# hitfeelee/rtm3d

Measured on AMD Instinct MI355X. Metric: images_per_sec, higher is better.
Workload: dtype fp16

## Files before the change

rtm3d_amd/csrc/common.h:

```cpp
#pragma once
#include <hip/hip_runtime.h>
#include <stdint.h>
#include <stddef.h>

typedef _Float16 f16;
typedef _Float16 f16x8 __attribute__((ext_vector_type(8)));
typedef _Float16 f16x4 __attribute__((ext_vector_type(4)));
typedef _Float16 f16x2 __attribute__((ext_vector_type(2)));
typedef float f32x4 __attribute__((ext_vector_type(4)));
typedef uint32_t u32x4 __attribute__((ext_vector_type(4)));

__device__ __forceinline__ int div_small_q(int m, int d, float rcp_d) {
    const int q = (int)((float)m * rcp_d);
    const int r = m - q * d;
    return q + (r >= d ? 1 : 0) - (r < 0 ? 1 : 0);
}


#define RT_DMA16(gptr, lds_byte_addr) \
    asm volatile("s_mov_b32 m0, %1\n\ts_nop 0\n\tglobal_load_lds_dwordx4 %0, off" : : "v"(gptr), "s"(lds_byte_addr) : "memory", "m0")
#define RT_DMA16_NT(gptr, lds_byte_addr) \
    asm volatile("s_mov_b32 m0, %1\n\ts_nop 0\n\tglobal_load_lds_dwordx4 %0, off nt" : : "v"(gptr), "s"(lds_byte_addr) : "memory", "m0")
static __device__ __forceinline__ const void* rt_uniform_ptr(const void* p) {
    const unsigned long long v = (unsigned long long)p;
// ... 151 lines not shown
    int in_coff[RT_MAX_GROUPS], out_coff[RT_MAX_GROUPS];
    int tap_pix[RT_MAX_TAPS];
};
struct QuantMx8Args {
    const f16* in;
    uint8_t* out;
    uint8_t* out_s;
    int B, H, W;
    int in_Hp, in_Wp, in_C, in_P, in_coff;
    int out_Hp, out_Wp, out_C, out_P, out_coff;
    int nblk;
};

struct PersistentGrid { int grid, single; };
inline PersistentGrid persistent_grid(int total, int cu_count) { return {cu_count < total ? cu_count : total, total <= cu_count ? 1 : 0}; }

hipError_t launch_patch_mask(const PatchMaskArgs& a, hipStream_t s);
hipError_t launch_conv32s2_fused(const Conv32S2Args& a, int cu_count, unsigned int* ticket_ctr, hipStream_t s);
hipError_t launch_stem_fused(const StemFusedArgs& a, hipStream_t s);
hipError_t launch_conv_headout(const HeadOutArgs& a, hipStream_t s);
hipError_t launch_conv_mfma(const ConvKArgs& a, int bn_tile, int groups, int epi_nchw, hipStream_t s);
hipError_t launch_conv_mfma_deep(const ConvKArgs& a, int bn_tile, int groups, unsigned int* tile_ctr, hipStream_t s);
hipError_t launch_conv_mfma256(const ConvKArgs& a, int groups, unsigned int* tile_ctr, float* stat_out, hipStream_t s);
enum Conv256Route { C256_ONE_TILE, C256_PERSISTENT, C256_HALO, C256_LATTICE };
Conv256Route conv_mfma256_route(const ConvKArgs& a, int groups, HaloTaps* ht);
void conv_mfma256_permute_weights(const f16* src, f16* dst, size_t n_ktiles);
bool conv64_halo_supported(const ConvKArgs& a, int groups);
hipError_t launch_conv64_halo(const ConvKArgs& a, int cu_count, unsigned int* ticket_ctr, hipStream_t s);
hipError_t launch_conv64_root(const ConvKArgs& a, const RootKArgs& r, int cu_count, unsigned int* ticket_ctr, hipStream_t s);
bool conv64s2_halo_supported(const ConvKArgs& a, int groups);
hipError_t launch_conv64s2_halo(const ConvKArgs& a, int cu_count, unsigned int* ticket_ctr, hipStream_t s);
bool conv128_halo_supported(const ConvKArgs& a, int groups);
hipError_t launch_conv128_halo(const ConvKArgs& a, int cu_count, unsigned int* ticket_ctr, hipStream_t s);
hipError_t launch_conv_smallc(const ConvKArgs& a, hipStream_t s);
bool conv_smallc_supported(int cin, int cout, int ntaps);
hipError_t launch_nchw_to_nhwc4(const float* in, f16* out, int B, int H, int W, int Hp, int Wp, int P, hipStream_t s);
hipError_t launch_maxpool(const PoolKArgs& a, hipStream_t s);
hipError_t launch_softmax_fuse(const SoftmaxKArgs& a, hipStream_t s);
hipError_t launch_quant_mx8(const QuantMx8Args& a, hipStream_t s);
hipError_t launch_conv_mx8(const ConvMx8Args& a, int groups, hipStream_t s);
```

rtm3d_amd/csrc/conv128_halo.hip:

```cpp
#include "common.h"

#define LDS_AS __attribute__((address_space(3)))
#define C128_NSW 3
#define C128_DMA16 RT_DMA16
#define C128_LDS_F16X8(byte_addr) (*(const LDS_AS f16x8*)(uintptr_t)(byte_addr))

template <int RES>
__global__ __launch_bounds__(512) void conv128_halo_kernel(const ConvKArgs a, unsigned int* ticket_ctr, const int single) {
    constexpr int TW = 32, CT = 128;
    constexpr int HW = TW + 2;
    constexpr int HALO_PIECES = 10 * HW * 8;
    constexpr int XI = (HALO_PIECES + 511) / 512;
    constexpr int XBUF_PIECES = XI * 512;
    constexpr int WSLOT_PIECES = CT * 8;
    constexpr int WI = WSLOT_PIECES / 512;
    constexpr int WCN = CT / 64;
    constexpr int WPN = 8 / WCN;
    constexpr int ROWS = 8 / WPN;
    __shared__ __attribute__((aligned(128))) f16 lds[(2 * XBUF_PIECES + C128_NSW * WSLOT_PIECES) * 8];
    __shared__ int tk[3];
    const int tid = threadIdx.x;
    const int lane = tid & 63;
    const int wave = __builtin_amdgcn_readfirstlane(tid >> 6);
    const int wc = wave % WCN, wp = wave / WCN;
    const int frow = lane & 15, fk = lane >> 4;
    const ConvGroupArgs& g = a.g[0];

    const int Hm = a.HmWm / a.Wm;
    const int tiles_x = a.Wm / TW, tpi = tiles_x * (Hm >> 3);
    const int NT = a.cout / CT, cpt = a.cpt;
    const int total = (a.M / a.HmWm) * tpi * NT;

    uint32_t poff[XI];
#pragma unroll
    for (int i = 0; i < XI; ++i) {
        int p = i * 512 + tid;
        p = p < HALO_PIECES ? p : HALO_PIECES - 1;
        const int hq = p >> 3, hcs = p & 7;
// ... 9 lines not shown
        cur = blockIdx.x; nxt = nn = total;
    } else {
        if (tid == 0) tk[0] = (int)atomicAdd(ticket_ctr, 3u);
        __syncthreads();
        const int tk0 = __builtin_amdgcn_readfirstlane(tk[0]);
        cur = tk0; nxt = tk0 + 1; nn = tk0 + 2;
    }
    if (cur >= total) return;
    __syncthreads();

    auto halo_origin = [&](int v) -> const f16* {
        const int pt = v / NT;
        const int n = pt / tpi, r = pt - n * tpi;
        const int ty = r / tiles_x, tx = r - ty * tiles_x;
        return a.in + ((size_t)(n * a.in_Hp + ty * 8 - 1 + a.in_P) * a.in_Wp + tx * TW - 1 + a.in_P) * a.in_C + g.in_coff;
    };
    auto issue_x = [&](const f16* src, int xb, int i, uint32_t off) {
        C128_DMA16(src + off, __builtin_amdgcn_readfirstlane(lds_x + (uint32_t)((xb * XBUF_PIECES + i * 512 + wave * 64) * 16)));
    };
    auto issue_w = [&](int nt, int tap, int chunk, int slot) {
        const f16* src = wsrc + (size_t)((nt * 9 + tap) * cpt + chunk) * (CT * 64);
#pragma unroll
        for (int i = 0; i < WI; ++i)
            C128_DMA16(src + i * 512 * 8, __builtin_amdgcn_readfirstlane(lds_w + (uint32_t)((slot * WSLOT_PIECES + i * 512 + wave * 64) * 16)));
    };

    const uint32_t lane_px = (uint32_t)(((ROWS * wp + 1) * HW + frow + 1) * 128);
    const uint32_t ck_m = (uint32_t)((((frow + 0) ^ fk) & 7) << 4), ck_0 = (uint32_t)((((frow + 1) ^ fk) & 7) << 4),
                   ck_p = (uint32_t)((((frow + 2) ^ fk) & 7) << 4);
    const uint32_t lane_w = (uint32_t)((wc * 64 + frow) * 128);
    const uint32_t wk0 = (uint32_t)(((fk ^ (frow & 7)) & 7) << 4), wk1 = (uint32_t)((((4 + fk) ^ (frow & 7)) & 7) << 4);
    const f16 lo = a.relu ? (f16)0.f : (f16)(-__builtin_inff());
    const f16x4 lo4 = {lo, lo, lo, lo};
    const int so = (fk & 1) * 16 + (fk >> 1) * 8;

    {
        const f16* src = halo_origin(cur);
#pragma unroll
        for (int i = 0; i < XI; ++i) issue_x(src, 0, i, poff[i]);
        issue_w(cur % NT, 0, 0, 0);
        issue_w(cur % NT, 1, 0, 1);
    }
    asm volatile("s_waitcnt vmcnt(0)" ::: "memory");

    int it = 0;
    f32x4 acc[4][4];
    for (;;) {
#pragma unroll
        for (int c = 0; c < 4; ++c)
#pragma unroll
            for (int p = 0; p < 4; ++p) acc[c][p] = (f32x4){0.f, 0.f, 0.f, 0.f};
        const bool more = nxt < total;
        const int nt_cur = cur % NT, nt_nxt = more ? nxt % NT : nt_cur;
        const f16* const src_cur = halo_origin(cur);
        const f16* const src_nxt = more ? halo_origin(nxt) : src_cur;
#pragma unroll 1
        for (int chunk = 0; chunk < cpt; ++chunk) {
            const bool last = chunk + 1 == cpt;
            const f16* const src_next = last ? src_nxt : src_cur + 64 * (chunk + 1);
            const int nt_next = last ? nt_nxt : nt_cur, chunk_next = last ? 0 : chunk + 1;
            const int xb = chunk & 1;
            uint32_t hb = lds_x + (uint32_t)(xb * XBUF_PIECES * 16);
            asm volatile("" : "+v"(hb));
#pragma unroll
            for (int t = 0; t < 9; ++t) {
                asm volatile("s_waitcnt vmcnt(%0)" : : "n"(WI + 1) : "memory");
                __builtin_amdgcn_sched_barrier(0);
                __builtin_amdgcn_s_barrier();
                __builtin_amdgcn_sched_barrier(0);
                if (chunk == 0 && t == 0 && it > 0) nn = __builtin_amdgcn_readfirstlane(tk[(it - 1) & 1]);
                {
                    if (t + 2 < 9) issue_w(nt_cur, t + 2, chunk, (t + 2) % C128_NSW);
                    else issue_w(nt_next, t + 2 - 9, chunk_next, (t + 2) % C128_NSW);
                    const int i = t < XI ? t : XI - 1;
                    issue_x(src_next, xb ^ 1, i, poff[i]);
                }
                const int dy = t / 3 - 1, dx = t % 3 - 1;
                const uint32_t ck = dx < 0 ? ck_m : (dx > 0 ? ck_p : ck_0);
                const uint32_t xt0 = hb + lane_px + (uint32_t)((dy * HW + dx) * 128) + ck;
                const uint32_t xu = xt0 ^ (uint32_t)(((1 + dy) & 1) << 6), xw = xu ^ 64u;
                const uint32_t wb = lds_w + (uint32_t)((t % C128_NSW) * WSLOT_PIECES * 16) + lane_w;
                f16x8 xf[2][4], wf[2][4];
#pragma unroll
                for (int kk = 0; kk < 2; ++kk) {
#pragma unroll
                    for (int p = 0; p < 4; ++p) {
                        const int prow = p >> 1, pcol = (p & 1) * 16;
                        const uint32_t ad = (((prow & 1) ^ kk) ? xw : xu) + (uint32_t)((prow * HW + pcol) * 128);
                        xf[kk][p] = C128_LDS_F16X8(ad);
                    }
#pragma unroll
                    for (int c = 0; c < 4; ++c) wf[kk][c] = C128_LDS_F16X8(wb + (uint32_t)(c * 16 * 128) + (kk ? wk1 : wk0));
                }
#pragma unroll
                for (int kk = 0; kk < 2; ++kk)
#pragma unroll
                    for (int c = 0; c < 4; ++c)
#pragma unroll
                        for (int p = 0; p < 4; ++p)
                            acc[c][p] = __builtin_amdgcn_mfma_f32_16x16x32_f16(wf[kk][c], xf[kk][p], acc[c][p], 0, 0, 0);
            }
        }
        if (!single && tid == 0) tk[it & 1] = (int)atomicAdd(ticket_ctr, 1u);

        {
            const int pt = cur / NT;
            const int n = pt / tpi, r = pt - n * tpi;
            const int ty = r / tiles_x, tx = r - ty * tiles_x;
            const int cbase = nt_cur * CT + wc * 64;
            f32x4 bv[4];
#pragma unroll
            for (int c = 0; c < 4; ++c) bv[c] = *(const f32x4*)(a.bias + g.bias_off + cbase + c * 16 + fk * 4);
            size_t opix[4];
            f16x4 rv[4][4];
#pragma unroll
            for (int p = 0; p < 4; ++p) {
                const int prow = p >> 1, pcol = (p & 1) * 16;
                const int oy = ty * 8 + ROWS * wp + prow, ox = tx * TW + pcol + frow;
                opix[p] = ((size_t)(n * a.out_Hp + oy + a.out_P) * a.out_Wp + ox + a.out_P) * a.out_C + g.out_coff + cbase;
                if (RES) {
                    const f16* rp = a.res + ((size_t)(n * a.res_Hp + oy + a.res_P) * a.res_Wp + ox + a.res_P) * a.res_C + g.res_coff + cbase + fk * 4;
#pragma unroll
                    for (int c = 0; c < 4; ++c) rv[p][c] = *(const f16x4*)(rp + c * 16);
                }
            }
#pragma unroll
            for (int p = 0; p < 4; ++p) {
                uint32_t u[4][2];
#pragma unroll
                for (int c = 0; c < 4; ++c) {
                    f32x4 v = acc[c][p] + bv[c];
                    if (RES) {
                        const f16x4 rr = rv[p][c];
                        v[0] += (float)rr[0]; v[1] += (float)rr[1]; v[2] += (float)rr[2]; v[3] += (float)rr[3];
                    }
                    f16x4 h = {(f16)v[0], (f16)v[1], (f16)v[2], (f16)v[3]};
                    h = __builtin_elementwise_max(h, lo4);
                    __builtin_memcpy(u[c], &h, 8);
                }
#pragma unroll
                for (int c = 0; c < 4; c += 2) {
                    const auto s0 = __builtin_amdgcn_permlane16_swap(u[c][0], u[c + 1][0], false, false);
                    const auto s1 = __builtin_amdgcn_permlane16_swap(u[c][1], u[c + 1][1], false, false);
                    const u32x4 o = {s0[0], s1[0], s0[1], s1[1]};
                    *(u32x4*)((f16*)a.out + opix[p] + c * 16 + so) = o;
                }
            }
        }
        if (!more) break;
        cur = nxt; nxt = nn;
        ++it;
    }
}

bool conv128_halo_supported(const ConvKArgs& a, int groups) {
    if (groups != 1 || a.cin % 128 || a.cout % 128 || a.ntaps != 9 || a.in_stride != 1 || a.out_scale != 1 || a.in_P < 1) return false;
    if (a.Wm % 32 || (a.HmWm / a.Wm) % 8 || a.M % a.HmWm) return false;
    const int pitch = a.in_Wp * a.in_C;
    for (int t = 0; t < 9; ++t)
        if (a.g[0].tap_off[t] != (t / 3 - 1) * pitch + (t % 3 - 1) * a.in_C) return false;
    return true;
}

hipError_t launch_conv128_halo(const ConvKArgs& a, int cu_count, unsigned int* ticket_ctr, hipStream_t s) {
    const int total = (a.M / a.HmWm) * (a.Wm >> 5) * ((a.HmWm / a.Wm) >> 3) * (a.cout / 128);
    const auto [grid, single] = persistent_grid(total, cu_count);
    if (a.res) hipLaunchKernelGGL(conv128_halo_kernel<1>, dim3(grid), dim3(512), 0, s, a, ticket_ctr, single);
    else hipLaunchKernelGGL(conv128_halo_kernel<0>, dim3(grid), dim3(512), 0, s, a, ticket_ctr, single);
    return hipGetLastError();
}
```

rtm3d_amd/csrc/conv_mfma256.hip:

```cpp
#include <string.h>
#include "common.h"

#define LDS_AS __attribute__((address_space(3)))
#define GLB_AS __attribute__((address_space(1)))

void conv_mfma256_permute_weights(const f16* src, f16* dst, size_t n_ktiles) {
    for (size_t k = 0; k < n_ktiles; ++k)
        for (int rd = 0; rd < 256; ++rd) {
            const int j = rd >> 7, wc = (rd >> 5) & 3, c = (rd >> 4) & 1, frow = rd & 15;
            const int rs = wc * 64 + frow * 4 + j * 2 + c;
            for (int pos = 0; pos < 8; ++pos) {
                const int chunk = pos ^ (rd & 7);
                memcpy(dst + (k * 256 + rd) * 64 + pos * 8, src + (k * 256 + rs) * 64 + (chunk ^ (rs & 7)) * 8, 16);
            }
        }
}

#define HALF_ELEMS (128 * 64)
#define BUF_ELEMS (4 * HALF_ELEMS)
#define SLOT_XA 0
#define SLOT_XB 1
#define SLOT_WA 2
#define SLOT_WB 3

__device__ __forceinline__ void c256_next_pixel(int& n, int& y, int& x, bool live, int Wm, int Hm) {
    const bool wx = x + 1 == Wm, wy = wx && y + 1 == Hm;
    const int x1 = wx ? 0 : x + 1, y1 = wy ? 0 : (wx ? y + 1 : y), n1 = wy ? n + 1 : n;
    x = live ? x1 : x; y = live ? y1 : y; n = live ? n1 : n;
}

template <int RES>
__global__ __launch_bounds__(512) void conv_mfma256_kernel(const ConvKArgs a) {
    __shared__ __attribute__((aligned(16))) f16 lds[2 * BUF_ELEMS + HALF_ELEMS];
    const int tid = threadIdx.x;
    const int lane = tid & 63;
    const int wave = __builtin_amdgcn_readfirstlane(tid >> 6);
    const int wp = wave & 1, wc = wave >> 1;

    const int bid = blockIdx.x;
    const int xcd = bid & 7, jb = bid >> 3;
    const int chunk = (a.MT + 7) >> 3;
    const int ntile = jb % a.NT;
    const int mtile = xcd * chunk + jb / a.NT;
    if (mtile >= a.MT) return;
    const ConvGroupArgs& g = a.g[blockIdx.y];
    const int T = a.ksteps;

    uint32_t xoff[2][2];
    {
        const int rr = tid >> 3, cs = tid & 7;
#pragma unroll
        for (int h = 0; h < 2; ++h)
#pragma unroll
            for (int i = 0; i < 2; ++i) {
                int m = mtile * 256 + h * 128 + i * 64 + rr;
                m = m < a.M ? m : a.M - 1;
                const int n = m / a.HmWm, rem = m - n * a.HmWm;
                const int y = rem / a.Wm, x = rem - y * a.Wm;
                const uint32_t pix = (uint32_t)((n * a.in_Hp + y * a.in_stride + a.in_P) * a.in_Wp + x * a.in_stride + a.in_P);
                xoff[h][i] = pix * (uint32_t)a.in_C + (uint32_t)g.in_coff + (uint32_t)((cs ^ (rr & 7)) * 8);
            }
    }
    const f16* wbase = a.wgt + g.w_off + (size_t)ntile * T * (256 * 64);
    f16* const dummy = lds + 2 * BUF_ELEMS;
// ... 74 lines not shown
        LOAD_W(wa, buf + SLOT_WA * HALF_ELEMS)
        stage(SLOT_WB, t + 1);
        SEG_SYNC()
        MMA(0, 0, wa)
        LOAD_W(wb, buf + SLOT_WB * HALF_ELEMS)
        stage(SLOT_XB, t + 1);
        SEG_SYNC()
        MMA(0, 1, wb)
        LOAD_X(buf + SLOT_XB * HALF_ELEMS)
        stage(SLOT_XA, t + 2);
        SEG_SYNC()
        MMA(1, 1, wb)
        stage(SLOT_WA, t + 2);
        SEG_SYNC()
        MMA(1, 0, wa)
    }
    if (wave < 4) __builtin_amdgcn_s_barrier();

    const f32x4 bv = *(const f32x4*)(a.bias + g.bias_off + ntile * 256 + wc * 64 + frow * 4);
    const float lo = a.relu ? 0.f : -__builtin_inff();
    const int cbase = ntile * 256 + wc * 64 + frow * 4;
    const int Hm = a.HmWm / a.Wm;
#pragma unroll
    for (int i = 0; i < 2; ++i) {
        size_t opix[4][4];
        f16x4 rv[4][4];
#pragma unroll
        for (int p = 0; p < 4; ++p) {
            const int m0 = mtile * 256 + i * 128 + wp * 64 + p * 16 + fk * 4;
            const int m = m0 < a.M ? m0 : a.M - 1;
            int n = m / a.HmWm;
            const int rem = m - n * a.HmWm;
            int y = rem / a.Wm, x = rem - y * a.Wm;
#pragma unroll
            for (int e = 0; e < 4; ++e) {
                if (e) c256_next_pixel(n, y, x, m0 + e < a.M, a.Wm, Hm);
                const int oy = y * a.out_scale + g.out_oy, ox = x * a.out_scale + g.out_ox;
                opix[p][e] = ((size_t)(n * a.out_Hp + oy + a.out_P) * a.out_Wp + ox + a.out_P) * a.out_C + g.out_coff + cbase;
                if (RES) rv[p][e] = *(const f16x4*)(a.res + ((size_t)(n * a.res_Hp + oy + a.res_P) * a.res_Wp + ox + a.res_P) * a.res_C + g.res_coff + cbase);
            }
        }
#pragma unroll
        for (int p = 0; p < 4; ++p)
#pragma unroll
            for (int e = 0; e < 4; ++e) {
                f32x4 v = {acc[i][0][0][p][e], acc[i][0][1][p][e], acc[i][1][0][p][e], acc[i][1][1][p][e]};
                v += bv;
                if (RES) {
                    const f16x4 r = rv[p][e];
                    v[0] += (float)r[0]; v[1] += (float)r[1]; v[2] += (float)r[2]; v[3] += (float)r[3];
                }
                const f16x4 h = {(f16)fmaxf(v[0], lo), (f16)fmaxf(v[1], lo), (f16)fmaxf(v[2], lo), (f16)fmaxf(v[3], lo)};
                *(f16x4*)((f16*)a.out + opix[p][e]) = h;
            }
    }
}

#define CONV256_MAX_BIAS 2048
#define DMA16 RT_DMA16
#define DMA16_NT RT_DMA16_NT
#define DMA16_SBASE RT_DMA16_SBASE
#define DMA16_SBASE_NT RT_DMA16_SBASE_NT
#define LDS_F16X8(byte_addr) (*(const LDS_AS f16x8*)(uintptr_t)(byte_addr))
#define LOAD_X_N(SLOT)                                                                      \
    _Pragma("unroll") for (int p = 0; p < 4; ++p) {                                         \
        xf[p][0] = LDS_F16X8(xaddr0 + (SLOT) * HALF_ELEMS * 2 + p * 2048);                  \
        xf[p][1] = LDS_F16X8(xaddr1 + (SLOT) * HALF_ELEMS * 2 + p * 2048);                  \
    }
#define LOAD_W_N(dstf, SLOT)                                                                \
    _Pragma("unroll") for (int c = 0; c < 2; ++c) {                                         \
        dstf[c][0] = LDS_F16X8(waddr0 + (SLOT) * HALF_ELEMS * 2 + c * 2048);                \
        dstf[c][1] = LDS_F16X8(waddr1 + (SLOT) * HALF_ELEMS * 2 + c * 2048);                \
// ... 79 lines not shown
    {                                                                                       \
         \
        const uint32_t xaddr0 = opa[0], xaddr1 = opa[1], waddr0 = opa[2], waddr1 = opa[3];  \
        LOAD_X_N(SLOT_XA)                                                                   \
        LOAD_W_N(wa, SLOT_WA)                                                               \
        STAGE_WB_P1                                                                         \
        SEG_SYNC_S(VM1, 0)                                                                  \
        MMA_S(0, 0, wa, FIRST, 1, 0)                                                        \
        LOAD_W_N(wb, SLOT_WB)                                                               \
        stage(SLOT_XB, t + 1, sp ^ 1, koff1);                                               \
        STAGE_WB_P2                                                                         \
        SEG_SYNC_S(VM, 5)                                                                   \
        MMA_S(0, 1, wb, FIRST, 1, 5)                                                        \
        LOAD_X_N(SLOT_XB)                                                                   \
        stage(SLOT_XA, t + 2, sp, koff2);                                                   \
        SEG_SYNC_S(VM, 10)                                                                  \
        MMA_S(1, 1, wb, FIRST, 1, 10)                                                       \
         \
              \
        int kchan3;                                                                         \
        int kraw3 = koff_parts(t + 3, kchan3);                                              \
        stage(SLOT_WA, t + 2, sp, 0);                                                       \
        OPA_SET(sp ^ 1)                                                                     \
        asm volatile("" : "+v"(opa[0]), "+v"(opa[1]), "+v"(opa[2]), "+v"(opa[3]));          \
        STAGE_WB_P4                                                                         \
        SEG_SYNC_S(VM, 15)                                                                  \
        asm volatile("" : "+s"(kraw3));            \
        const int koff3 = kraw3 + kchan3;                                                   \
        MMA_S(1, 0, wa, FIRST, !(LAST), 15)                                                 \
        koff1 = koff2; koff2 = koff3;                                                       \
        sp ^= 1;                                                                            \
    }

template <int RES, int XNT>
__global__ __launch_bounds__(512) void conv_mfma256_persistent_kernel(const ConvKArgs a, const int groups, const int nbias, unsigned int* tile_ctr, const int one_list) {
    __shared__ __attribute__((aligned(16))) f16 lds[2 * BUF_ELEMS + HALF_ELEMS];
    __shared__ __attribute__((aligned(16))) float lds_bias[CONV256_MAX_BIAS + 4];
#ifdef C256_STAMPS
    __shared__ unsigned long long lds_stamp[2][C256_STAMP_KT][C256_STAMP_N];
    __shared__ unsigned long long lds_tstamp[2][4][4];
    int stamp_tile = 0;
#endif
    const int tid = threadIdx.x;
    const int lane = tid & 63;
    const int wave = __builtin_amdgcn_readfirstlane(tid >> 6);
    const int wp = wave & 1, wc = wave >> 1;
    const int T = a.ksteps;
    for (int i = tid; i < nbias; i += 512) lds_bias[i] = a.bias[i];
    __syncthreads();

    const int xcd = one_list ? 0 : blockIdx.x & 7, per_xcd = one_list ? gridDim.x : gridDim.x >> 3;
    const int chunk = one_list ? a.MT : (a.MT + 7) >> 3;
    int mt_here = a.MT - xcd * chunk;
    mt_here = mt_here < 0 ? 0 : (mt_here > chunk ? chunk : mt_here);
    const int jbs = mt_here * a.NT;
    const int vtotal = jbs * groups;
    int* const lds_ticket = (int*)(lds_bias + CONV256_MAX_BIAS);
    const int last_draw = vtotal + per_xcd - 1;
    if (tid == 0) {
        const int t0 = (int)atomicAdd(&tile_ctr[xcd], 1u);
        if (t0 == last_draw) tile_ctr[xcd] = 0u;
        lds_ticket[0] = t0;
    }
    __syncthreads();
    const int v = __builtin_amdgcn_readfirstlane(lds_ticket[0]);
    if (v >= vtotal) return;

// ... 134 lines not shown
        }
        int t = 0;
        TSTAMP(0)
        if (first_tile) STEP_N(8, VM1_8, 1, 0) else STEP_N(40, VM1_40, 1, 0)
        first_tile = false;
        if (wave == 0) {
            asm volatile("s_waitcnt vmcnt(8)" : "+v"(ticket) : : "memory");
            if (lane == 0) {
                lds_ticket[tpar] = ticket;
                if (draw && ticket == last_draw) tile_ctr[xcd] = 0u;
            }
        }
        live_n = draw;
        if (live_n) locate(vnext, xo_n, wb_n, gi_n, mt_n, nt_n);
        for (t = 1; t < T - 1; ++t) STEP_N(8, VM1_8, 0, 0)
        STEP_N(8, VM1_8, 0, 1)
        if (wave < 4) __builtin_amdgcn_s_barrier();
        TSTAMP(1)

        {
            const ConvGroupArgs& g = a.g[gi_c];
            const int cbase = nt_c * 256 + wc * 64 + frow * 4;
#pragma unroll
            for (int i = 0; i < 2; ++i) {
                size_t opix[4][4];
                f16x4 rv[4][4];
#pragma unroll
                for (int p = 0; p < 4; ++p) {
                    const int m0 = mt_c * 256 + i * 128 + wp * 64 + p * 16 + fk * 4;
                    const int m = m0 < a.M ? m0 : a.M - 1;
                    int n = div_small_q(m, a.HmWm, rcp_hw);
                    const int rem = m - n * a.HmWm;
                    int y = div_small_q(rem, a.Wm, rcp_w), x = rem - y * a.Wm;
#pragma unroll
                    for (int e = 0; e < 4; ++e) {
                        if (e) c256_next_pixel(n, y, x, m0 + e < a.M, a.Wm, Hm);
                        const int oy = y * a.out_scale + g.out_oy, ox = x * a.out_scale + g.out_ox;
                        opix[p][e] = ((size_t)(n * a.out_Hp + oy + a.out_P) * a.out_Wp + ox + a.out_P) * a.out_C + g.out_coff + cbase;
                        if (RES) rv[p][e] = *(const f16x4*)(a.res + ((size_t)(n * a.res_Hp + oy + a.res_P) * a.res_Wp + ox + a.res_P) * a.res_C + g.res_coff + cbase);
                    }
                }
#pragma unroll
                for (int p = 0; p < 4; ++p)
#pragma unroll
                    for (int e = 0; e < 4; ++e) {
                        f32x4 vv = {acc[i][0][0][p][e], acc[i][0][1][p][e], acc[i][1][0][p][e], acc[i][1][1][p][e]};
                        if (RES) {
                            const f16x4 r = rv[p][e];
                            vv[0] += (float)r[0]; vv[1] += (float)r[1]; vv[2] += (float)r[2]; vv[3] += (float)r[3];
                        }
                        f16x4 h = {(f16)vv[0], (f16)vv[1], (f16)vv[2], (f16)vv[3]};
                        h = __builtin_elementwise_max(h, lo4);
                        *(f16x4*)((f16*)a.out + opix[p][e]) = h;
                    }
            }
        }
        TSTAMP(2)
        if (wave >= 4) __builtin_amdgcn_s_barrier();
        TSTAMP(3)
#ifdef C256_STAMPS
        ++stamp_tile;
#endif
        if (!live_n) break;
        vnext = __builtin_amdgcn_readfirstlane(lds_ticket[tpar]);
        tpar ^= 1;
        xo_c[0][0] = xo_n[0][0]; xo_c[0][1] = xo_n[0][1]; xo_c[1][0] = xo_n[1][0]; xo_c[1][1] = xo_n[1][1];
        wb_c = wb_n; gi_c = gi_n; mt_c = mt_n; nt_c = nt_n;
    }
    if (wave < 4) __builtin_amdgcn_s_barrier();
#ifdef C256_STAMPS
    if ((blockIdx.x == 0 || blockIdx.x == 101) && (wave & 3) == 0) {
        asm volatile("s_waitcnt vmcnt(0) lgkmcnt(0)" ::: "memory");
// ... 20 lines not shown
    }
    return n;
}

static int conv256_nbias(const ConvKArgs& a, int groups) {
    int nbias = 0;
    for (int g = 0; g < groups; ++g) nbias = a.g[g].bias_off + a.cout > nbias ? a.g[g].bias_off + a.cout : nbias;
    return (nbias + 255) / 256 * 256;
}

Conv256Route conv_mfma256_route(const ConvKArgs& a, int groups, HaloTaps* ht) {
    const int nbias = conv256_nbias(a, groups);
    const unsigned long long in_bytes = (unsigned long long)(a.M / a.HmWm) * a.in_Hp * a.in_Wp * a.in_C * 2ull;
    if (a.ksteps < 4 || nbias > CONV256_MAX_BIAS || in_bytes >= (1ull << 32)) return C256_ONE_TILE;
    HaloTaps scratch;
    if (!ht) ht = &scratch;
#ifdef C256_T_NOHALO9
    if (a.ntaps == 9) {} else
#endif
    if (!a.res && (a.ntaps == 9 || a.ntaps == 4) && nbias <= 1024 && conv_mfma256_halo_supported(a, groups, ht)) return C256_HALO;
#ifndef C256_T_NOLATTICE
    if (nbias <= 1024 && conv_mfma256_lattice_dilation(a, groups) != 0) return C256_LATTICE;
#endif
    return C256_PERSISTENT;
}

hipError_t launch_conv_mfma256(const ConvKArgs& a, int groups, unsigned int* tile_ctr, float* stat_out, hipStream_t s) {
    dim3 block(512, 1, 1);
    HaloTaps ht;
    const Conv256Route route = conv_mfma256_route(a, groups, &ht);
    if (stat_out && route != C256_HALO) return hipErrorInvalidValue;
    if (route != C256_ONE_TILE && !tile_ctr) return hipErrorInvalidValue;
    const int nbias = conv256_nbias(a, groups);
    if (route == C256_HALO) return launch_conv_mfma256_halo(a, ht, groups, nbias, device_cu_count(), tile_ctr, stat_out, s);
    if (route == C256_LATTICE) return launch_conv_mfma256_lattice(a, groups, nbias, device_cu_count(), tile_ctr, s);
    if (route == C256_PERSISTENT) {
        const int per_xcd = device_cu_count() / 8;
        const int one_list = (long long)a.MT * a.NT * groups <= device_cu_count() ? 1 : 0;
        dim3 grid(per_xcd * 8, 1, 1);
        const bool x_once = !a.res && a.ntaps == 1 && a.NT == 1 && a.in_stride == 1;
        if (a.res) hipLaunchKernelGGL((conv_mfma256_persistent_kernel<1, 0>), grid, block, 0, s, a, groups, nbias, tile_ctr, one_list);
        else if (x_once) hipLaunchKernelGGL((conv_mfma256_persistent_kernel<0, 1>), grid, block, 0, s, a, groups, nbias, tile_ctr, one_list);
        else hipLaunchKernelGGL((conv_mfma256_persistent_kernel<0, 0>), grid, block, 0, s, a, groups, nbias, tile_ctr, one_list);
        return hipGetLastError();
    }
    const int mt8 = (a.MT + 7) / 8 * 8;
    dim3 grid(mt8 * a.NT, groups, 1);
    if (a.res) hipLaunchKernelGGL((conv_mfma256_kernel<1>), grid, block, 0, s, a);
    else hipLaunchKernelGGL((conv_mfma256_kernel<0>), grid, block, 0, s, a);
    return hipGetLastError();
}
```

rtm3d_amd/csrc/runtime.hip:

```cpp
#include <math.h>
#include <stdarg.h>
#include <stdio.h>
#include <string.h>
#include <string>
#include <vector>

#include "common.h"
#include "../../include/rtm3d_hip.h"

static thread_local char g_err[512] = "";
void rt_set_error(const char* fmt, ...) {
    va_list ap;
    va_start(ap, fmt);
    vsnprintf(g_err, sizeof(g_err), fmt, ap);
    va_end(ap);
}
#define RT_FAIL(...) do { rt_set_error(__VA_ARGS__); return 1; } while (0)
#define RT_HIP(expr) do { hipError_t e_ = (expr); if (e_ != hipSuccess) { rt_set_error("%s: %s", #expr, hipGetErrorString(e_)); return 1; } } while (0)

struct Tensor {
    int B, H, W, C, P, Hp, Wp;
    f16* alloc;
    f16* base;
    size_t elems;
// ... 191 lines not shown
    RT_HIP(hipMemcpy(p, h_data, bytes, hipMemcpyHostToDevice));
    ctx->blobs.push_back(p);
    ctx->blob_bytes.push_back(bytes);
    *id = (int)ctx->blobs.size() - 1;
    return 0;
}

extern "C" int rtm3d_tensor_info(rtm3d_ctx* ctx, int id, void** d_base, int* B, int* H, int* W, int* C, int* border) {
    Tensor* t = ctx ? get_tensor(ctx, id) : nullptr;
    if (!t) RT_FAIL("tensor_info: bad tensor %d", id);
    if (d_base) *d_base = t->base;
    if (B) *B = t->B;
    if (H) *H = t->H;
    if (W) *W = t->W;
    if (C) *C = t->C;
    if (border) *border = t->P;
    return 0;
}

static void* get_blob(rtm3d_ctx* ctx, int id, size_t* bytes);
extern "C" int rtm3d_blob_address(rtm3d_ctx* ctx, int id, void** d_ptr, size_t* bytes) {
    void* p = ctx ? get_blob(ctx, id, bytes) : nullptr;
    if (!p || !d_ptr) RT_FAIL("blob_address: bad blob %d", id);
    *d_ptr = p;
    return 0;
}

static void* get_blob(rtm3d_ctx* ctx, int id, size_t* bytes) {
    if (id < 0 || id >= (int)ctx->blobs.size()) return nullptr;
    if (bytes) *bytes = ctx->blob_bytes[id];
    return ctx->blobs[id];
}

static int admit_mfma128(rtm3d_ctx* ctx, const rtm3d_conv_desc* d, size_t wbytes, size_t bbytes, Op& op) {
    ConvKArgs& a = op.conv;
    const int BN = d->bn_tile;
    if (BN != 16 && BN != 32 && BN != 64 && BN != 128) RT_FAIL("op_conv: bn_tile must be 16/32/64/128");
    if (d->cin % 64) RT_FAIL("op_conv(mfma): cin=%d is not a multiple of 64", d->cin);
    if (!d->out_nchw_f32 && (d->cout % BN)) RT_FAIL("op_conv(mfma): cout=%d is not a multiple of the tile %d", d->cout, BN);
    if (d->out_nchw_f32 && a.res) RT_FAIL("op_conv(mfma): the NCHW fp32 epilogue adds no residual");
    const int cout_pad = (d->cout + BN - 1) / BN * BN;
    a.cpt = d->cin / 64; a.ksteps = d->ntaps * a.cpt;
    a.MT = (a.M + 127) / 128; a.NT = cout_pad / BN;
    const size_t per_group = (size_t)cout_pad * a.ksteps * 64;
    if (wbytes != per_group * d->groups * sizeof(f16)) RT_FAIL("op_conv(mfma): packed weight blob has %zu bytes, expected %zu", wbytes, per_group * d->groups * sizeof(f16));
    if (bbytes != (size_t)cout_pad * d->groups * sizeof(float)) RT_FAIL("op_conv(mfma): bias blob has %zu bytes, expected %zu", bbytes, (size_t)cout_pad * d->groups * sizeof(float));
    for (int g = 0; g < d->groups; ++g) { a.g[g].w_off = (uint32_t)(per_group * g); a.g[g].bias_off = cout_pad * g; }
    op.kind = OP_CONV_MFMA; op.bn_tile = BN;
    op.name = d->ntaps == 1 ? "conv1x1_mfma" : (d->ntaps == 4 ? "deconv4x4_phase_mfma" : "conv3x3_mfma");
    if (d->out_nchw_f32 || (BN != 64 && BN != 128)) return 0;
    const long long wgs = (long long)a.MT * a.NT * d->groups;
    if (wgs > ctx->n_cus) return 0;
    a.deep = 1;
    op.name += "_deep";
    if (ensure_tile_ctr(ctx)) return 1;
    if (wgs * 2 > ctx->n_cus || wgs > SPLIT_CTRS || a.ksteps < 8) return 0;
    int ks = (int)(ctx->n_cus / wgs);
    if (ks > a.ksteps / 4) ks = a.ksteps / 4;
    if (ks > 16) ks = 16;
    if (ks < 2) return 0;
    const size_t need = (size_t)ks * wgs * 128 * BN;
    if (need > ctx->slab_floats) {
        float* nslab = nullptr;
        RT_HIP(hipMalloc((void**)&nslab, need * sizeof(float)));
        ctx->extra.push_back(nslab);
        for (auto& prev : ctx->ops) if (prev.kind == OP_CONV_MFMA && prev.conv.ksplit > 1) prev.conv.slab = nslab;
        ctx->slab = nslab; ctx->slab_floats = need;
    }
    a.ksplit = ks; a.slab = ctx->slab;
    op.name += "_splitk";
    return 0;
}

static int admit_mfma256(rtm3d_ctx* ctx, const rtm3d_conv_desc* d, size_t wbytes, size_t bbytes, Op& op) {
    ConvKArgs& a = op.conv;
    if (d->cin % 64 || d->cout % 256 || d->out_nchw_f32) RT_FAIL("op_conv(mfma256): needs cin %% 64 == 0, cout %% 256 == 0, NHWC output (cin=%d cout=%d)", d->cin, d->cout);
    a.cpt = d->cin / 64; a.ksteps = d->ntaps * a.cpt;
    a.MT = (a.M + 255) / 256; a.NT = d->cout / 256;
    const size_t per_group = (size_t)d->cout * a.ksteps * 64;
    if (wbytes != per_group * d->groups * sizeof(f16)) RT_FAIL("op_conv(mfma256): packed weight blob has %zu bytes, expected %zu", wbytes, per_group * d->groups * sizeof(f16));
    if (bbytes != (size_t)d->cout * d->groups * sizeof(float)) RT_FAIL("op_conv(mfma256): bias blob size mismatch");
    for (int g = 0; g < d->groups; ++g) { a.g[g].w_off = (uint32_t)(per_group * g); a.g[g].bias_off = d->cout * g; }
    op.kind = OP_CONV_MFMA256; op.bn_tile = 256;
    if (ensure_tile_ctr(ctx)) return 1;
    {
        std::vector<f16> h_src(wbytes / sizeof(f16)), h_dst(wbytes / sizeof(f16));
        RT_HIP(hipMemcpy(h_src.data(), a.wgt, wbytes, hipMemcpyDeviceToHost));
        conv_mfma256_permute_weights(h_src.data(), h_dst.data(), wbytes / (256 * 64 * sizeof(f16)));
        f16* w_perm = nullptr;
        RT_HIP(hipMalloc((void**)&w_perm, wbytes + 256));
        ctx->extra.push_back(w_perm);
        RT_HIP(hipMemset(w_perm, 0, wbytes + 256));
        RT_HIP(hipMemcpy(w_perm, h_dst.data(), wbytes, hipMemcpyHostToDevice));
        a.wgt = w_perm;
    }
    static const char* const suffix[] = {"_1tile", "", "_halo", "_lattice"};
    op.name = d->ntaps == 1 ? "conv1x1_mfma256" : (d->ntaps == 4 ? "deconv4x4_phase_mfma256" : "conv3x3_mfma256");
    op.name += suffix[conv_mfma256_route(a, d->groups, nullptr)];
    return 0;
}

static int admit_smallc(rtm3d_ctx*, const rtm3d_conv_desc* d, size_t wbytes, size_t bbytes, Op& op) {
    ConvKArgs& a = op.conv;
    if (d->groups != 1) RT_FAIL("op_conv(smallc): groups=%d unsupported (one group)", d->groups);
    if (d->out_nchw_f32) RT_FAIL("op_conv(smallc): NCHW output unsupported");
    if (a.res) RT_FAIL("op_conv(smallc): residual unsupported");
    if (!conv_smallc_supported(d->cin, d->cout, d->ntaps)) RT_FAIL("op_conv(smallc): no kernel for cin=%d cout=%d ntaps=%d", d->cin, d->cout, d->ntaps);
    int S = d->cin == 16 ? 5 : (d->cin == 32 ? d->ntaps : 7);
    if (d->cin == 16 && d->cout == 16 && d->in_stride == 1 && d->out_scale == 1 && wbytes == (size_t)(d->cout / 16) * 6 * 64 * 8 * sizeof(f16)) S = 6;
    if (wbytes != (size_t)(d->cout / 16) * S * 64 * 8 * sizeof(f16)) RT_FAIL("op_conv(smallc): weight blob size mismatch");
    a.ksteps = S;
    if (bbytes != (size_t)d->cout * sizeof(float)) RT_FAIL("op_conv(smallc): bias blob size mismatch");
    if (d->cin == 4 && a.in_P < 4) RT_FAIL("op_conv(smallc): the NHWC4 stem input needs a border of 4");
    if (d->cin == 4 && (a.in_C != 4 || d->in_coff[0] != 0)) RT_FAIL("op_conv(smallc): cin=4 reads a 4-channel NHWC4 tensor (input tensor has %d channels, in_coff=%d)", a.in_C, d->in_coff[0]);
    if (d->cin != 4 && a.in_C % 8) RT_FAIL("op_conv(smallc): 16-byte operand loads are misaligned in an input tensor of %d channels (needs a multiple of 8)", a.in_C);
    if (d->cout != 16 && a.out_C % 8) RT_FAIL("op_conv(smallc): 16-byte stores are misaligned in an output tensor of %d channels (needs a multiple of 8)", a.out_C);
    const int* dy = d->tap_dy[0];
    const int* dx = d->tap_dx[0];
    const bool rows = d->in_stride == 1 && d->out_scale == 1 && d->cout == 16 && (d->cin == 4 || (d->cin == 16 && S == 6));
    if (rows) {
        const int K = d->cin == 4 ? 7 : 3;
        for (int t = 0; t < d->ntaps; ++t)
            if (dy[t] != dy[0] + t / K || dx[t] != dx[0] + t % K)
                RT_FAIL("op_conv(smallc): tap geometry: the vertical-walk kernel needs the dense %dx%d taps in row-major order, dilation 1 (tap %d is (%d,%d), expected (%d,%d))",
                        K, K, t, dy[t], dx[t], dy[0] + t / K, dx[0] + t % K);
    } else if (d->cin == 4) {
        for (int t = 0; t < d->ntaps; ++t)
            if (t % 7 && (dy[t] != dy[t - 1] || dx[t] != dx[t - 1] + 1))
// ... 2 lines not shown
    }
    if (d->cin == 4)
        for (int ky = 0; ky < 7; ++ky)
            if ((d->Wm - 1) * d->in_stride + dx[ky * 7 + 6] + 1 >= a.in_Wp - a.in_P)
                RT_FAIL("op_conv(smallc): the pixel right of tap (%d,%d), read with zero weight, leaves the padded input", dy[ky * 7 + 6], dx[ky * 7 + 6]);
    a.g[0].w_off = 0; a.g[0].bias_off = 0;
    op.kind = OP_CONV_SMALLC;
    op.name = d->cin == 4 ? "stem7x7_regmfma" : "conv_smallc_regmfma";
    return 0;
}

static int admit_c64_halo(rtm3d_ctx* ctx, const rtm3d_conv_desc* d, size_t wbytes, size_t bbytes, Op& op) {
    ConvKArgs& a = op.conv;
    if (d->out_nchw_f32) RT_FAIL("op_conv(conv64): NCHW output unsupported");
    if (!a.out) RT_FAIL("op_conv: writing ONLY the space-to-depth copy needs kernel 0");
    a.cpt = 1; a.ksteps = 9; a.MT = 0; a.NT = 1;
    if (!conv64_halo_supported(a, d->groups)) RT_FAIL("op_conv(conv64): needs one 64->64 3x3 stride-1 conv on a map with W %% 32 == 0, H %% 8 == 0");
    if (wbytes != (size_t)9 * 64 * 64 * sizeof(f16) || bbytes != 64 * sizeof(float)) RT_FAIL("op_conv(conv64): weight/bias blob size mismatch");
    if (claim_ticket(ctx, op, "op_conv(conv64)")) return 1;
    a.g[0].w_off = 0; a.g[0].bias_off = 0;
    op.kind = OP_CONV64_HALO; op.bn_tile = 64;
    op.name = "conv3x3_c64_halo";
    return 0;
}

static int admit_c128_halo(rtm3d_ctx* ctx, const rtm3d_conv_desc* d, size_t wbytes, size_t bbytes, Op& op) {
    ConvKArgs& a = op.conv;
    if (d->out_nchw_f32) RT_FAIL("op_conv(conv128): NCHW output unsupported");
    a.cpt = d->cin / 64; a.ksteps = 9 * a.cpt; a.MT = 0; a.NT = 1;
    if (!conv128_halo_supported(a, d->groups)) RT_FAIL("op_conv(conv128): needs one 3x3 stride-1 conv with cin, cout %% 128 == 0 on a map with W %% 32 == 0, H %% 8 == 0");
    if (d->bn_tile != 128 || wbytes != (size_t)9 * d->cin * d->cout * sizeof(f16) || bbytes != (size_t)d->cout * sizeof(float))
        RT_FAIL("op_conv(conv128): weight/bias blob size mismatch (expects the bn_tile = 128 packing)");
    if (claim_ticket(ctx, op, "op_conv(conv128)")) return 1;
    a.g[0].w_off = 0; a.g[0].bias_off = 0;
    op.kind = OP_CONV128_HALO; op.bn_tile = 128;
    op.name = "conv3x3_c128_halo";
    return 0;
}

static int admit_c64s2_halo(rtm3d_ctx* ctx, const rtm3d_conv_desc* d, size_t wbytes, size_t bbytes, Op& op) {
    ConvKArgs& a = op.conv;
    if (d->in_s2d) {
        if (d->groups != 1) RT_FAIL("op_conv: a space-to-depth INPUT is read by kernel 7 only");
        if (!slice_ok(d->in_coff[0], 4 * d->cin, a.in_C) || a.in_P < 1) RT_FAIL("op_conv: the space-to-depth input needs 4 x cin channels behind in_coff and a border >= 1");
    }
    if (d->out_nchw_f32 || a.res) RT_FAIL("op_conv(conv64s2): NCHW output / residual unsupported");
    a.cpt = 1; a.ksteps = 9; a.MT = 0; a.NT = 1;
    a.in_s2d = d->in_s2d ? 1 : 0;
    if (!conv64s2_halo_supported(a, d->groups)) RT_FAIL("op_conv(conv64s2): needs one 64->128 3x3 stride-2 conv onto a map with W %% 32 == 0, H %% 4 == 0 (input border >= 1)");
    if (wbytes != (size_t)9 * 64 * 128 * sizeof(f16) || bbytes != 128 * sizeof(float)) RT_FAIL("op_conv(conv64s2): weight/bias blob size mismatch");
    if (claim_ticket(ctx, op, "op_conv(conv64s2)")) return 1;
    a.g[0].w_off = 0; a.g[0].bias_off = 0;
    op.kind = OP_CONV64S2_HALO; op.bn_tile = 128;
    op.name = "conv3x3s2_c64_halo";
    return 0;
}

extern "C" int rtm3d_op_conv(rtm3d_ctx* ctx, const rtm3d_conv_desc* d) {
    if (!ctx || !d) RT_FAIL("op_conv: null argument");
    Tensor* in = get_tensor(ctx, d->in_tensor);
    if (d->s2d_tensor < 0) RT_FAIL("op_conv: s2d_tensor = %d (tensor id + 1, 0 = none)", d->s2d_tensor);
    const int s2d_id = d->s2d_tensor - 1;
    const bool s2d_only = !d->out_nchw_f32 && d->out_tensor < 0 && s2d_id >= 0;
    Tensor* out = (d->out_nchw_f32 || s2d_only) ? nullptr : get_tensor(ctx, d->out_tensor);
    Tensor* res = d->res_tensor >= 0 ? get_tensor(ctx, d->res_tensor) : nullptr;
    if (!in) RT_FAIL("op_conv: bad input tensor %d", d->in_tensor);
// ... 845 lines not shown
```

Baseline: 2719.

## Transpose MFMA operands in conv128 halo and add row-contiguous epilogue for conv256

For the 128-channel halo conv, the output-channel rows of the weights are permuted once on the host at admission, and the MFMA operands are swapped so each lane holds four consecutive channels for four pixels. The epilogue can then store f16x4 per pixel directly, with no permlane16 swaps, and the bias load shrinks to one vector. Separately, the mfma256 kernels gain a ROW4 variant: when the map width, pixels-per-image and M are all multiples of 4, the output and residual addresses for the 4 consecutive pixels come from a fixed stride instead of per-pixel div/mod index math. The cost is narrower 8-byte stores spread across pixels instead of 16-byte stores, plus more template instantiations.

```diff
diff --git a/rtm3d_amd/csrc/common.h b/rtm3d_amd/csrc/common.h
--- a/rtm3d_amd/csrc/common.h
+++ b/rtm3d_amd/csrc/common.h
@@ -207,6 +207,7 @@
 hipError_t launch_conv64s2_halo(const ConvKArgs& a, int cu_count, unsigned int* ticket_ctr, hipStream_t s);
 bool conv128_halo_supported(const ConvKArgs& a, int groups);
 hipError_t launch_conv128_halo(const ConvKArgs& a, int cu_count, unsigned int* ticket_ctr, hipStream_t s);
+void conv128_halo_permute_weights(const f16* src, f16* dst, size_t n_ktiles);
 hipError_t launch_conv_smallc(const ConvKArgs& a, hipStream_t s);
 bool conv_smallc_supported(int cin, int cout, int ntaps);
 hipError_t launch_nchw_to_nhwc4(const float* in, f16* out, int B, int H, int W, int Hp, int Wp, int P, hipStream_t s);
diff --git a/rtm3d_amd/csrc/conv128_halo.hip b/rtm3d_amd/csrc/conv128_halo.hip
--- a/rtm3d_amd/csrc/conv128_halo.hip
+++ b/rtm3d_amd/csrc/conv128_halo.hip
@@ -1,9 +1,22 @@
+#include <string.h>
 #include "common.h"
 
 #define LDS_AS __attribute__((address_space(3)))
 #define C128_NSW 3
 #define C128_DMA16 RT_DMA16
 #define C128_LDS_F16X8(byte_addr) (*(const LDS_AS f16x8*)(uintptr_t)(byte_addr))
+
+void conv128_halo_permute_weights(const f16* src, f16* dst, size_t n_ktiles) {
+    for (size_t k = 0; k < n_ktiles; ++k)
+        for (int rd = 0; rd < 128; ++rd) {
+            const int wc = rd >> 6, c = (rd >> 4) & 3, frow = rd & 15;
+            const int rs = wc * 64 + frow * 4 + c;
+            for (int pos = 0; pos < 8; ++pos) {
+                const int chunk = pos ^ (rd & 7);
+                memcpy(dst + (k * 128 + rd) * 64 + pos * 8, src + (k * 128 + rs) * 64 + (chunk ^ (rs & 7)) * 8, 16);
+            }
+        }
+}
 
 template <int RES>
 __global__ __launch_bounds__(512) void conv128_halo_kernel(const ConvKArgs a, unsigned int* ticket_ctr, const int single) {
@@ -79,7 +92,6 @@
     const uint32_t wk0 = (uint32_t)(((fk ^ (frow & 7)) & 7) << 4), wk1 = (uint32_t)((((4 + fk) ^ (frow & 7)) & 7) << 4);
     const f16 lo = a.relu ? (f16)0.f : (f16)(-__builtin_inff());
     const f16x4 lo4 = {lo, lo, lo, lo};
-    const int so = (fk & 1) * 16 + (fk >> 1) * 8;
 
     {
         const f16* src = halo_origin(cur);
@@ -145,7 +157,7 @@
                     for (int c = 0; c < 4; ++c)
 #pragma unroll
                         for (int p = 0; p < 4; ++p)
-                            acc[c][p] = __builtin_amdgcn_mfma_f32_16x16x32_f16(wf[kk][c], xf[kk][p], acc[c][p], 0, 0, 0);
+                            acc[c][p] = __builtin_amdgcn_mfma_f32_16x16x32_f16(xf[kk][p], wf[kk][c], acc[c][p], 0, 0, 0);
             }
         }
         if (!single && tid == 0) tk[it & 1] = (int)atomicAdd(ticket_ctr, 1u);
@@ -154,45 +166,35 @@
             const int pt = cur / NT;
             const int n = pt / tpi, r = pt - n * tpi;
             const int ty = r / tiles_x, tx = r - ty * tiles_x;
-            const int cbase = nt_cur * CT + wc * 64;
-            f32x4 bv[4];
-#pragma unroll
-            for (int c = 0; c < 4; ++c) bv[c] = *(const f32x4*)(a.bias + g.bias_off + cbase + c * 16 + fk * 4);
+            const int cbase = nt_cur * CT + wc * 64 + frow * 4;
+            const f32x4 bv = *(const f32x4*)(a.bias + g.bias_off + cbase);
             size_t opix[4];
             f16x4 rv[4][4];
 #pragma unroll
             for (int p = 0; p < 4; ++p) {
                 const int prow = p >> 1, pcol = (p & 1) * 16;
-                const int oy = ty * 8 + ROWS * wp + prow, ox = tx * TW + pcol + frow;
+                const int oy = ty * 8 + ROWS * wp + prow, ox = tx * TW + pcol + fk * 4;
                 opix[p] = ((size_t)(n * a.out_Hp + oy + a.out_P) * a.out_Wp + ox + a.out_P) * a.out_C + g.out_coff + cbase;
                 if (RES) {
-                    const f16* rp = a.res + ((size_t)(n * a.res_Hp + oy + a.res_P) * a.res_Wp + ox + a.res_P) * a.res_C + g.res_coff + cbase + fk * 4;
-#pragma unroll
-                    for (int c = 0; c < 4; ++c) rv[p][c] = *(const f16x4*)(rp + c * 16);
+                    const f16* rp = a.res + ((size_t)(n * a.res_Hp + oy + a.res_P) * a.res_Wp + ox + a.res_P) * a.res_C + g.res_coff + cbase;
+#pragma unroll
+                    for (int e = 0; e < 4; ++e) rv[p][e] = *(const f16x4*)(rp + (size_t)e * a.res_C);
                 }
             }
 #pragma unroll
-            for (int p = 0; p < 4; ++p) {
-                uint32_t u[4][2];
-#pragma unroll
-                for (int c = 0; c < 4; ++c) {
-                    f32x4 v = acc[c][p] + bv[c];
+            for (int p = 0; p < 4; ++p)
+#pragma unroll
+                for (int e = 0; e < 4; ++e) {
+                    f32x4 v = {acc[0][p][e], acc[1][p][e], acc[2][p][e], acc[3][p][e]};
+                    v += bv;
                     if (RES) {
-                        const f16x4 rr = rv[p][c];
+                        const f16x4 rr = rv[p][e];
                         v[0] += (float)rr[0]; v[1] += (float)rr[1]; v[2] += (float)rr[2]; v[3] += (float)rr[3];
                     }
                     f16x4 h = {(f16)v[0], (f16)v[1], (f16)v[2], (f16)v[3]};
                     h = __builtin_elementwise_max(h, lo4);
-                    __builtin_memcpy(u[c], &h, 8);
-                }
-#pragma unroll
-                for (int c = 0; c < 4; c += 2) {
-                    const auto s0 = __builtin_amdgcn_permlane16_swap(u[c][0], u[c + 1][0], false, false);
-                    const auto s1 = __builtin_amdgcn_permlane16_swap(u[c][1], u[c + 1][1], false, false);
-                    const u32x4 o = {s0[0], s1[0], s0[1], s1[1]};
-                    *(u32x4*)((f16*)a.out + opix[p] + c * 16 + so) = o;
-                }
-            }
+                    *(f16x4*)((f16*)a.out + opix[p] + (size_t)e * a.out_C) = h;
+                }
         }
         if (!more) break;
         cur = nxt; nxt = nn;
diff --git a/rtm3d_amd/csrc/conv_mfma256.hip b/rtm3d_amd/csrc/conv_mfma256.hip
--- a/rtm3d_amd/csrc/conv_mfma256.hip
+++ b/rtm3d_amd/csrc/conv_mfma256.hip
@@ -29,7 +29,13 @@
     x = live ? x1 : x; y = live ? y1 : y; n = live ? n1 : n;
 }
 
-template <int RES>
+__device__ __forceinline__ void c256_row4_steps(const ConvKArgs& a, int m0, size_t& ostep, size_t& rstep) {
+    const bool live = m0 < a.M;
+    ostep = live ? (size_t)(a.out_scale * a.out_C) : 0;
+    rstep = live ? (size_t)(a.out_scale * a.res_C) : 0;
+}
+
+template <int RES, int ROW4>
 __global__ __launch_bounds__(512) void conv_mfma256_kernel(const ConvKArgs a) {
     __shared__ __attribute__((aligned(16))) f16 lds[2 * BUF_ELEMS + HALF_ELEMS];
     const int tid = threadIdx.x;
@@ -170,12 +176,23 @@
             int n = m / a.HmWm;
             const int rem = m - n * a.HmWm;
             int y = rem / a.Wm, x = rem - y * a.Wm;
+            size_t ostep = 0, rstep = 0;
+            const f16* rbase = a.res;
+            if (ROW4) c256_row4_steps(a, m0, ostep, rstep);
 #pragma unroll
             for (int e = 0; e < 4; ++e) {
+                if (ROW4 && e) {
+                    opix[p][e] = opix[p][0] + e * ostep;
+                    if (RES) rv[p][e] = *(const f16x4*)(rbase + e * rstep);
+                    continue;
+                }
                 if (e) c256_next_pixel(n, y, x, m0 + e < a.M, a.Wm, Hm);
                 const int oy = y * a.out_scale + g.out_oy, ox = x * a.out_scale + g.out_ox;
                 opix[p][e] = ((size_t)(n * a.out_Hp + oy + a.out_P) * a.out_Wp + ox + a.out_P) * a.out_C + g.out_coff + cbase;
-                if (RES) rv[p][e] = *(const f16x4*)(a.res + ((size_t)(n * a.res_Hp + oy + a.res_P) * a.res_Wp + ox + a.res_P) * a.res_C + g.res_coff + cbase);
+                if (RES) {
+                    rbase = a.res + ((size_t)(n * a.res_Hp + oy + a.res_P) * a.res_Wp + ox + a.res_P) * a.res_C + g.res_coff + cbase;
+                    rv[p][e] = *(const f16x4*)rbase;
+                }
             }
         }
 #pragma unroll
@@ -321,7 +338,7 @@
         sp ^= 1;                                                                            \
     }
 
-template <int RES, int XNT>
+template <int RES, int XNT, int ROW4>
 __global__ __launch_bounds__(512) void conv_mfma256_persistent_kernel(const ConvKArgs a, const int groups, const int nbias, unsigned int* tile_ctr, const int one_list) {
     __shared__ __attribute__((aligned(16))) f16 lds[2 * BUF_ELEMS + HALF_ELEMS];
     __shared__ __attribute__((aligned(16))) float lds_bias[CONV256_MAX_BIAS + 4];
@@ -522,12 +539,23 @@
                     int n = div_small_q(m, a.HmWm, rcp_hw);
                     const int rem = m - n * a.HmWm;
                     int y = div_small_q(rem, a.Wm, rcp_w), x = rem - y * a.Wm;
+                    size_t ostep = 0, rstep = 0;
+                    const f16* rbase = a.res;
+                    if (ROW4) c256_row4_steps(a, m0, ostep, rstep);
 #pragma unroll
                     for (int e = 0; e < 4; ++e) {
+                        if (ROW4 && e) {
+                            opix[p][e] = opix[p][0] + e * ostep;
+                            if (RES) rv[p][e] = *(const f16x4*)(rbase + e * rstep);
+                            continue;
+                        }
                         if (e) c256_next_pixel(n, y, x, m0 + e < a.M, a.Wm, Hm);
                         const int oy = y * a.out_scale + g.out_oy, ox = x * a.out_scale + g.out_ox;
                         opix[p][e] = ((size_t)(n * a.out_Hp + oy + a.out_P) * a.out_Wp + ox + a.out_P) * a.out_C + g.out_coff + cbase;
-                        if (RES) rv[p][e] = *(const f16x4*)(a.res + ((size_t)(n * a.res_Hp + oy + a.res_P) * a.res_Wp + ox + a.res_P) * a.res_C + g.res_coff + cbase);
+                        if (RES) {
+                            rbase = a.res + ((size_t)(n * a.res_Hp + oy + a.res_P) * a.res_Wp + ox + a.res_P) * a.res_C + g.res_coff + cbase;
+                            rv[p][e] = *(const f16x4*)rbase;
+                        }
                     }
                 }
 #pragma unroll
@@ -614,6 +642,7 @@
     if (stat_out && route != C256_HALO) return hipErrorInvalidValue;
     if (route != C256_ONE_TILE && !tile_ctr) return hipErrorInvalidValue;
     const int nbias = conv256_nbias(a, groups);
+    const bool row4 = a.Wm % 4 == 0 && a.HmWm % 4 == 0 && a.M % 4 == 0;
     if (route == C256_HALO) return launch_conv_mfma256_halo(a, ht, groups, nbias, device_cu_count(), tile_ctr, stat_out, s);
     if (route == C256_LATTICE) return launch_conv_mfma256_lattice(a, groups, nbias, device_cu_count(), tile_ctr, s);
     if (route == C256_PERSISTENT) {
@@ -621,14 +650,16 @@
         const int one_list = (long long)a.MT * a.NT * groups <= device_cu_count() ? 1 : 0;
         dim3 grid(per_xcd * 8, 1, 1);
         const bool x_once = !a.res && a.ntaps == 1 && a.NT == 1 && a.in_stride == 1;
-        if (a.res) hipLaunchKernelGGL((conv_mfma256_persistent_kernel<1, 0>), grid, block, 0, s, a, groups, nbias, tile_ctr, one_list);
-        else if (x_once) hipLaunchKernelGGL((conv_mfma256_persistent_kernel<0, 1>), grid, block, 0, s, a, groups, nbias, tile_ctr, one_list);
-        else hipLaunchKernelGGL((conv_mfma256_persistent_kernel<0, 0>), grid, block, 0, s, a, groups, nbias, tile_ctr, one_list);
+#define C256_LAUNCH_P(RES, XNT, ROW4) hipLaunchKernelGGL((conv_mfma256_persistent_kernel<RES, XNT, ROW4>), grid, block, 0, s, a, groups, nbias, tile_ctr, one_list)
+        if (a.res) { if (row4) C256_LAUNCH_P(1, 0, 1); else C256_LAUNCH_P(1, 0, 0); }
+        else if (x_once) { if (row4) C256_LAUNCH_P(0, 1, 1); else C256_LAUNCH_P(0, 1, 0); }
+        else { if (row4) C256_LAUNCH_P(0, 0, 1); else C256_LAUNCH_P(0, 0, 0); }
+#undef C256_LAUNCH_P
         return hipGetLastError();
     }
     const int mt8 = (a.MT + 7) / 8 * 8;
     dim3 grid(mt8 * a.NT, groups, 1);
-    if (a.res) hipLaunchKernelGGL((conv_mfma256_kernel<1>), grid, block, 0, s, a);
-    else hipLaunchKernelGGL((conv_mfma256_kernel<0>), grid, block, 0, s, a);
+    if (a.res) { if (row4) hipLaunchKernelGGL((conv_mfma256_kernel<1, 1>), grid, block, 0, s, a); else hipLaunchKernelGGL((conv_mfma256_kernel<1, 0>), grid, block, 0, s, a); }
+    else { if (row4) hipLaunchKernelGGL((conv_mfma256_kernel<0, 1>), grid, block, 0, s, a); else hipLaunchKernelGGL((conv_mfma256_kernel<0, 0>), grid, block, 0, s, a); }
     return hipGetLastError();
 }
diff --git a/rtm3d_amd/csrc/runtime.hip b/rtm3d_amd/csrc/runtime.hip
--- a/rtm3d_amd/csrc/runtime.hip
+++ b/rtm3d_amd/csrc/runtime.hip
@@ -247,6 +247,19 @@
     return ctx->blobs[id];
 }
 
+static int permuted_weight_copy(rtm3d_ctx* ctx, ConvKArgs& a, size_t wbytes, int tile_rows, void (*permute)(const f16*, f16*, size_t)) {
+    std::vector<f16> h_src(wbytes / sizeof(f16)), h_dst(wbytes / sizeof(f16));
+    RT_HIP(hipMemcpy(h_src.data(), a.wgt, wbytes, hipMemcpyDeviceToHost));
+    permute(h_src.data(), h_dst.data(), wbytes / ((size_t)tile_rows * 64 * sizeof(f16)));
+    f16* w_perm = nullptr;
+    RT_HIP(hipMalloc((void**)&w_perm, wbytes + 256));
+    ctx->extra.push_back(w_perm);
+    RT_HIP(hipMemset(w_perm, 0, wbytes + 256));
+    RT_HIP(hipMemcpy(w_perm, h_dst.data(), wbytes, hipMemcpyHostToDevice));
+    a.wgt = w_perm;
+    return 0;
+}
+
 static int admit_mfma128(rtm3d_ctx* ctx, const rtm3d_conv_desc* d, size_t wbytes, size_t bbytes, Op& op) {
     ConvKArgs& a = op.conv;
     const int BN = d->bn_tile;
@@ -298,17 +311,7 @@
     for (int g = 0; g < d->groups; ++g) { a.g[g].w_off = (uint32_t)(per_group * g); a.g[g].bias_off = d->cout * g; }
     op.kind = OP_CONV_MFMA256; op.bn_tile = 256;
     if (ensure_tile_ctr(ctx)) return 1;
-    {
-        std::vector<f16> h_src(wbytes / sizeof(f16)), h_dst(wbytes / sizeof(f16));
-        RT_HIP(hipMemcpy(h_src.data(), a.wgt, wbytes, hipMemcpyDeviceToHost));
-        conv_mfma256_permute_weights(h_src.data(), h_dst.data(), wbytes / (256 * 64 * sizeof(f16)));
-        f16* w_perm = nullptr;
-        RT_HIP(hipMalloc((void**)&w_perm, wbytes + 256));
-        ctx->extra.push_back(w_perm);
-        RT_HIP(hipMemset(w_perm, 0, wbytes + 256));
-        RT_HIP(hipMemcpy(w_perm, h_dst.data(), wbytes, hipMemcpyHostToDevice));
-        a.wgt = w_perm;
-    }
+    if (permuted_weight_copy(ctx, a, wbytes, 256, conv_mfma256_permute_weights)) return 1;
     static const char* const suffix[] = {"_1tile", "", "_halo", "_lattice"};
     op.name = d->ntaps == 1 ? "conv1x1_mfma256" : (d->ntaps == 4 ? "deconv4x4_phase_mfma256" : "conv3x3_mfma256");
     op.name += suffix[conv_mfma256_route(a, d->groups, nullptr)];
@@ -377,6 +380,7 @@
     if (d->bn_tile != 128 || wbytes != (size_t)9 * d->cin * d->cout * sizeof(f16) || bbytes != (size_t)d->cout * sizeof(float))
         RT_FAIL("op_conv(conv128): weight/bias blob size mismatch (expects the bn_tile = 128 packing)");
     if (claim_ticket(ctx, op, "op_conv(conv128)")) return 1;
+    if (permuted_weight_copy(ctx, a, wbytes, 128, conv128_halo_permute_weights)) return 1;
     a.g[0].w_off = 0; a.g[0].bias_off = 0;
     op.kind = OP_CONV128_HALO; op.bn_tile = 128;
     op.name = "conv3x3_c128_halo";
```

Result: no change. 2741, median of 6 (+0.8%).
